# 10XGenomics/lariat

Hardware: AMD Instinct MI355X
Metric: read-pairs/sec aligned to hg38 (per-barcode align loop: SMEM seeding + SW + RFA/MAPQ on device); synthetic hg38-scale reference (higher is better)
Workload: dtype u64/i32 (FM-index + integer DP), f64 (RFA scores)

## Files before the change

### lariat_amd/csrc/k_chain.h

```cpp
#pragma once
#include "k_seed.h"
#include "lh_sort.h"

struct DChainTmp {
    i64 pos, last_rbeg;
    int32_t first_qbeg, last_qbeg, last_len, rid, n, head, tail, w, kept, first, beg, end;
};
#ifndef LH_CHAIN_LDS
#define LH_CHAIN_LDS 256
#endif
struct DChain {
    i64 pos;
    int32_t rid, n, seed_start, w, kept, is_alt;
    float frac_rep;
    int32_t pad;
};

__global__ void __launch_bounds__(64) k_chain(DIndex ix, DOpts o, int n_reads, const i64* __restrict__ seq_off, const i64* __restrict__ seed_off,
                                               i64 pool_cap, const DSeed* __restrict__ seeds, const int32_t* __restrict__ s_rid,
                                               const int32_t* __restrict__ l_rep, int32_t* __restrict__ s_next, DChainTmp* __restrict__ ct,
                                               int32_t* __restrict__ ord, int32_t* __restrict__ srt, DChain* __restrict__ chains,
                                               DSeed* __restrict__ cseeds, int32_t* __restrict__ n_chains, int32_t* __restrict__ status,
                                               const int32_t* __restrict__ list, const int32_t* __restrict__ list_count) {
    __shared__ DChainTmp Cs[LH_CHAIN_LDS];
// ... 215 lines not shown
            if (!shadowed) {
                if (lane == 0) { od[nk] = i; C[st[i]].kept = large_ovlp ? 2 : 3; }
                nk++;
                WAVE_SYNC();
            }
        }
        if (lane == 0) {
            for (int i = 0; i < nk; ++i) {
                int f = C[st[od[i]]].first;
                if (f >= 0) C[st[f]].kept = 1;
            }
            int i, k;
            for (i = k = 0; i < n; ++i) {
                int kp = C[st[i]].kept;
                if (kp == 0 || kp == 3) continue;
                if (++k >= o.max_chain_extend) break;
            }
            for (; i < n; ++i)
                if (C[st[i]].kept < 3) C[st[i]].kept = 0;
        }
    }
    WAVE_SYNC();
    int m = 0;
    {
        int sstart = 0;
        const float frac_rep = (float)l_rep[r] / len;
        for (int i0 = 0; i0 < n; i0 += 64) {
            const int i = i0 + lane;
            int kept = 0, cn = 0;
            DChainTmp c;
            if (i < n) { c = C[st[i]]; kept = c.kept != 0; cn = kept ? c.n : 0; }
            const u64 km = __ballot(kept);
            const int incl = wave_scan_add_i32(cn);
            if (kept) {
                DChain oc;
                oc.pos = c.pos; oc.rid = c.rid; oc.n = c.n; oc.seed_start = sstart + incl - cn; oc.w = c.w; oc.kept = c.kept; oc.is_alt = (ix.contig_alt && ix.contig_alt[c.rid]) ? 1 : 0;
                oc.frac_rep = frac_rep; oc.pad = st[i];
                chains[base + m + lanes_below(km, lane)] = oc;
            }
            m += (int)__popcll(km);
            sstart += wave_readlane(incl, 63);
        }
        if (lane == 0) n_chains[r] = m;
    }
    WAVE_SYNC();
    for (int k = lane; k < m; k += 64) {
        DChain oc = chains[base + k];
        int s = C[oc.pad].head;
        for (int t = 0; s >= 0; s = nx[s], ++t) cseeds[base + oc.seed_start + t] = sd_[s];
    }
    }
}

#ifndef LH_CHAIN_LANE_MAX
#define LH_CHAIN_LANE_MAX 32
#endif
#ifndef LH_EXT_HEAVY_COLS
#define LH_EXT_HEAVY_COLS 64
#endif
#ifndef LH_NARROW_MAX_LOSS
#define LH_NARROW_MAX_LOSS 36
#endif
```

### lariat_amd/csrc/k_chain_lane.h

```cpp
#pragma once
#include "k_extend2.h"

#ifndef LH_CHAIN_LANE_WAVES
#define LH_CHAIN_LANE_WAVES 2
#endif
#define LH_CHAIN_LANE_MAXC 8
#define CLW(ci_, f_) cl[(((ci_) << 3) + (f_)) * 64 + lane]
#define NIB(x_, i_) ((int)(((x_) >> ((i_) << 2)) & 0xf))
#define NIB_SET(x_, i_, v_) ((x_) = ((x_) & ~(0xfu << ((i_) << 2))) | ((uint32_t)(v_) << ((i_) << 2)))
template <class Lt> __device__ __forceinline__ void dev_introsort_small_nib(int n, uint32_t& a, Lt lt, int32_t* wdp) {
    if (n < 1) return;
    if (n == 2) {
        if (lt(NIB(a, 1), NIB(a, 0))) { int x = NIB(a, 0), y = NIB(a, 1); NIB_SET(a, 0, y); NIB_SET(a, 1, x); }
        return;
    }
    if (n > 1) {
        int t = n - 1, i = 0, j = t, k = i + ((j - i) >> 1) + 1;
        if (lt(NIB(a, k), NIB(a, i))) {
            if (lt(NIB(a, k), NIB(a, j))) k = j;
        } else k = lt(NIB(a, j), NIB(a, i)) ? i : j;
        const int rp = NIB(a, k);
        if (k != t) { int y = NIB(a, t); NIB_SET(a, k, y); NIB_SET(a, t, rp); }
        int wd = 4 * LH_CHAIN_LANE_MAX + 8;
        for (;;) {
            do { ++i; LH_WATCH(wdp, wd, 4, return) } while (lt(NIB(a, i), rp));
            do { --j; LH_WATCH(wdp, wd, 5, return) } while (i <= j && lt(rp, NIB(a, j)));
            if (j <= i) break;
            int x = NIB(a, i), y = NIB(a, j); NIB_SET(a, i, y); NIB_SET(a, j, x);
        }
        { int x = NIB(a, i), y = NIB(a, t); NIB_SET(a, i, y); NIB_SET(a, t, x); }
    }
    for (int i = 1; i < n; ++i)
        for (int j = i; j > 0 && lt(NIB(a, j), NIB(a, j - 1)); --j) { int x = NIB(a, j), y = NIB(a, j - 1); NIB_SET(a, j, y); NIB_SET(a, j - 1, x); }
}
__global__ void __launch_bounds__(64, LH_CHAIN_LANE_WAVES) k_chain_lane(DIndex ix, DOpts o, int n_reads, i64 pool_cap, const DSeed* __restrict__ seeds, const int32_t* __restrict__ s_rid,
                                                    const int32_t* __restrict__ l_rep, DChain* __restrict__ chains, DSeed* __restrict__ cseeds, int32_t* __restrict__ n_chains,
                                                    int32_t* __restrict__ status, int32_t* __restrict__ list, int32_t* __restrict__ list_count, int32_t* __restrict__ srt,
                                                    i64* __restrict__ chain_rmax, DCounters* __restrict__ ctr, ExtArgs A, int fuse,
                                                    int32_t* __restrict__ next_count, int32_t* __restrict__ next_list, int32_t* __restrict__ next_key,
                                                    int32_t* __restrict__ defer_count, int32_t* __restrict__ defer_list) {
    const i64* __restrict__ seq_off = A.seq_off; const i64* __restrict__ seed_off = A.seed_off; int32_t* __restrict__ sdone = A.sdone;
    __shared__ uint32_t cl[LH_CHAIN_LANE_MAXC * 8 * 64];
    const int r = blockIdx.x * blockDim.x + threadIdx.x, lane = LANE();
    int heavy = 0, ext_out = 0, ext_key = 0;
    u64 win = 0, cells = 0;
    int nch_done = 0;
    if (r < n_reads) {
        const i64 base = seed_off[r];
        const int S = (int)(seed_off[r + 1] - base);
        if (seed_off[r + 1] > pool_cap) { n_chains[r] = 0; A.n_regs[r] = 0; atomicOr(&status[r], LH_ST_POOL_OVERFLOW); }
        else if (S > LH_CHAIN_LANE_MAX) heavy = 1;
        else {
            const int len = (int)(seq_off[r + 1] - seq_off[r]);
            const DSeed* sd_ = seeds + base;
            const int32_t* rid_ = s_rid + base;
            int nch = 0;
            uint32_t od = 0;
            u64 smap0 = ~0ull, smap1 = ~0ull;
#define SMAP_SET(s_, v_) { if ((s_) < 16) smap0 = (smap0 & ~(0xfull << ((s_) << 2))) | ((u64)(v_) << ((s_) << 2)); else smap1 = (smap1 & ~(0xfull << (((s_) - 16) << 2))) | ((u64)(v_) << (((s_) - 16) << 2)); }
#define SMAP_GET(s_) ((int)((((s_) < 16 ? smap0 : smap1) >> (((s_) & 15) << 2)) & 0xf))
            DSeed pn; pn.rbeg = 0; pn.qbeg = 0; pn.len = 0;
            int ridn = -1;
            if (S > 0) { pn = sd_[0]; ridn = rid_[0]; }
            for (int s = 0; s < S && !heavy; ++s) {
                const DSeed p = pn;
                const int rid = ridn;
                if (s + 1 < S) { pn = sd_[s + 1]; ridn = rid_[s + 1]; }
                if (rid < 0) continue;
                int to_add = 1, lo = 0;
                for (int k = 0; k < nch; ++k) {
                    const int ci = NIB(od, k);
                    const i64 pos = (i64)((u64)CLW(ci, 0) | (u64)CLW(ci, 1) << 32);
                    if (pos <= p.rbeg) lo = k + 1; else break;
                }
                if (lo > 0) {
                    const int ci = NIB(od, lo - 1);
                    const i64 c_pos = (i64)((u64)CLW(ci, 0) | (u64)CLW(ci, 1) << 32);
                    const uint32_t qp = CLW(ci, 3), ridw = CLW(ci, 4);
                    const i64 c_last_rbeg = c_pos + (int32_t)CLW(ci, 2);
                    const int c_first_qbeg = qp & 0xff, c_last_qbeg = (qp >> 8) & 0xff, c_last_len = (qp >> 16) & 0xff, c_rid = (int)(ridw & 0x3fffffffu);
                    const i64 qend = c_last_qbeg + c_last_len, rend = c_last_rbeg + c_last_len;
                    int res = 0;
                    if (rid != c_rid) res = 0;
                    else if (p.qbeg >= c_first_qbeg && p.qbeg + p.len <= qend && p.rbeg >= c_pos && p.rbeg + p.len <= rend) res = 1;
                    else if ((c_last_rbeg < ix.l_pac || c_pos < ix.l_pac) && p.rbeg >= ix.l_pac) res = 0;
                    else {
                        i64 x = p.qbeg - c_last_qbeg, y = p.rbeg - c_last_rbeg;
                        if (y >= 0 && x - y <= o.w && y - x <= o.w && x - c_last_len < o.max_chain_gap && y - c_last_len < o.max_chain_gap) res = 2;
                    }
                    if (res == 2) {
                        const int rr = (int)(p.rbeg - c_pos);
                        CLW(ci, 2) = (uint32_t)rr;
                        CLW(ci, 3) = (uint32_t)c_first_qbeg | (uint32_t)p.qbeg << 8 | (uint32_t)p.len << 16;
                        uint32_t w5 = CLW(ci, 5), w6 = CLW(ci, 6);
                        int n = w5 & 0xff, wq = (int)(w5 >> 8), endq = w6 & 0xff, wr = (int)(w6 >> 8), endr = (int32_t)CLW(ci, 7);
                        if (p.qbeg >= endq) wq += p.len; else if (p.qbeg + p.len > endq) wq += p.qbeg + p.len - endq;
                        endq = endq > p.qbeg + p.len ? endq : p.qbeg + p.len;
                        if (rr >= endr) wr += p.len; else if (rr + p.len > endr) wr += rr + p.len - endr;
                        endr = endr > rr + p.len ? endr : rr + p.len;
                        CLW(ci, 5) = (uint32_t)(n + 1) | (uint32_t)wq << 8; CLW(ci, 6) = (uint32_t)endq | (uint32_t)wr << 8; CLW(ci, 7) = (uint32_t)endr;
                        SMAP_SET(s, ci)
                    }
                    to_add = (res == 0);
                }
                if (to_add) {
                    if (nch == LH_CHAIN_LANE_MAXC) { heavy = 1; break; }
                    const uint32_t lowm = lo ? (0xffffffffu >> (32 - (lo << 2))) : 0u;
                    od = (od & lowm) | ((uint32_t)nch << (lo << 2)) | ((lo < 7) ? ((od & ~lowm) << 4) : 0u);
                    CLW(nch, 0) = (uint32_t)(u64)p.rbeg; CLW(nch, 1) = (uint32_t)((u64)p.rbeg >> 32); CLW(nch, 2) = 0;
                    CLW(nch, 3) = (uint32_t)p.qbeg | (uint32_t)p.qbeg << 8 | (uint32_t)p.len << 16;
                    CLW(nch, 4) = (uint32_t)rid | ((ix.contig_alt && ix.contig_alt[rid]) ? 1u << 30 : 0u);
                    CLW(nch, 5) = 1u | (uint32_t)p.len << 8; CLW(nch, 6) = (uint32_t)(p.qbeg + p.len) | (uint32_t)p.len << 8; CLW(nch, 7) = (uint32_t)p.len;
                    SMAP_SET(s, nch)
                    nch++;
                }
            }
            if (!heavy) {
            for (int k = 0; k < nch; ++k) {
                const uint32_t w5 = CLW(k, 5), w6 = CLW(k, 6);
                int wq = (int)(w5 >> 8), wr = (int)(w6 >> 8);
                int w = wr < wq ? wr : wq;
                CLW(k, 6) = (uint32_t)(w < 1 << 30 ? w : (1 << 30) - 1);
                CLW(k, 5) = w5 & 0xff;
            }
#define C_W(id_) ((int)CLW(id_, 6))
#define C_BEG(id_) ((int)(CLW(id_, 3) & 0xff))
#define C_END(id_) ((int)(((CLW(id_, 3) >> 8) & 0xff) + ((CLW(id_, 3) >> 16) & 0xff)))
#define C_KEPT(id_) ((int)((CLW(id_, 5) >> 8) & 0xff))
#define C_SET_KEPT(id_, v_) (CLW(id_, 5) = (CLW(id_, 5) & ~0xff00u) | ((uint32_t)(v_) << 8))
#define C_FIRST(id_) ((int)((CLW(id_, 5) >> 16) & 0xff) - 1)
#define C_SET_FIRST(id_, v_) (CLW(id_, 5) = (CLW(id_, 5) & ~0xff0000u) | ((uint32_t)((v_) + 1) << 16))
            uint32_t st = 0;
            int n = 0;
            for (int k = 0; k < nch; ++k) {
                const int id = NIB(od, k);
                if (C_W(id) < o.min_chain_weight) continue;
                NIB_SET(st, n, id); n++;
            }
            if (n > 0) {
                dev_introsort_small_nib(n, st, [&](int x, int y) { return C_W(x) > C_W(y); }, o.wd);
                uint32_t kl = 0;
                int nk = 0;
                C_SET_KEPT(NIB(st, 0), 3);
                NIB_SET(kl, nk, 0); nk++;
                for (int i = 1; i < n; ++i) {
                    int large_ovlp = 0, k;
                    const int idi = NIB(st, i);
                    const int ai_beg = C_BEG(idi), ai_end = C_END(idi), ai_w = C_W(idi), ai_alt = (int)(CLW(idi, 4) >> 30) & 1;
                    for (k = 0; k < nk; ++k) {
                        const int idj = NIB(st, NIB(kl, k));
                        const int aj_beg = C_BEG(idj), aj_end = C_END(idj), aj_w = C_W(idj), aj_alt = (int)(CLW(idj, 4) >> 30) & 1;
                        int b_max = aj_beg > ai_beg ? aj_beg : ai_beg;
                        int e_min = aj_end < ai_end ? aj_end : ai_end;
                        if (e_min > b_max && (!aj_alt || ai_alt)) {
                            int li = ai_end - ai_beg, lj = aj_end - aj_beg;
                            int min_l = li < lj ? li : lj;
                            if (e_min - b_max >= min_l * o.mask_level && min_l < o.max_chain_gap) {
                                large_ovlp = 1;
                                if (C_FIRST(idj) < 0) C_SET_FIRST(idj, i);
                                if (ai_w < aj_w * o.drop_ratio && aj_w - ai_w >= o.min_seed_len << 1) break;
                            }
                        }
                    }
                    if (k == nk) { NIB_SET(kl, nk, i); nk++; C_SET_KEPT(idi, large_ovlp ? 2 : 3); }
                }
                for (int i = 0; i < nk; ++i) {
                    int f = C_FIRST(NIB(st, NIB(kl, i)));
                    if (f >= 0) C_SET_KEPT(NIB(st, f), 1);
                }
                int i, k;
                for (i = k = 0; i < n; ++i) {
                    int kp = C_KEPT(NIB(st, i));
                    if (kp == 0 || kp == 3) continue;
                    if (++k >= o.max_chain_extend) break;
                }
                for (; i < n; ++i)
                    if (C_KEPT(NIB(st, i)) < 3) C_SET_KEPT(NIB(st, i), 0);
            }
            int m = 0, sstart = 0;
            const float frac_rep = (float)l_rep[r] / len;
            for (int i = 0; i < n; ++i) {
                const int id = NIB(st, i);
                const int kp = C_KEPT(id);
                if (kp == 0) { CLW(id, 7) = 0xffffffffu; continue; }
                DChain oc;
                oc.pos = (i64)((u64)CLW(id, 0) | (u64)CLW(id, 1) << 32); oc.rid = (int)(CLW(id, 4) & 0x3fffffffu); oc.n = (int)(CLW(id, 5) & 0xff); oc.seed_start = sstart;
                oc.w = C_W(id); oc.kept = kp; oc.is_alt = (int)(CLW(id, 4) >> 30) & 1;
                oc.frac_rep = frac_rep; oc.pad = id;
                chains[base + m] = oc;
                CLW(id, 7) = (uint32_t)sstart; CLW(id, 2) = 0;
                sstart += oc.n;
                m++;
            }
            for (int k = 0; k < nch; ++k) if (C_W(k) < o.min_chain_weight) CLW(k, 7) = 0xffffffffu;
            for (int s = 0; s < S; ++s) {
                const int id = SMAP_GET(s);
                if (id == 0xf) continue;
                const uint32_t ss = CLW(id, 7);
                if (ss == 0xffffffffu) continue;
                const uint32_t t = CLW(id, 2);
                cseeds[base + ss + t] = sd_[s];
                CLW(id, 2) = t + 1;
            }
            n_chains[r] = m;
#undef SMAP_SET
#undef SMAP_GET
#undef C_W
#undef C_BEG
#undef C_END
#undef C_KEPT
#undef C_SET_KEPT
#undef C_FIRST
#undef C_SET_FIRST
            {
                int l_query = len > LH_MAXLEN ? 0 : len;
                const i64 l_pac = ix.l_pac;
                for (int ci = 0; ci < m; ++ci) {
                    DChain c = chains[base + ci];
                    const DSeed* sd = cseeds + base + c.seed_start;
                    int32_t* so = srt + base + c.seed_start;
                    int32_t* done = sdone + base + c.seed_start;
                    const int n = c.n;
                    if (n == 0) continue;
                    i64 r0 = l_pac << 1, r1 = 0;
                    for (int i = 0; i < n; ++i) {
                        DSeed t = sd[i];
                        i64 b = t.rbeg - (t.qbeg + dev_cal_max_gap(o, t.qbeg));
                        i64 e = t.rbeg + t.len + ((l_query - t.qbeg - t.len) + dev_cal_max_gap(o, l_query - t.qbeg - t.len));
                        r0 = r0 < b ? r0 : b;
                        r1 = r1 > e ? r1 : e;
                    }
                    i64 rmax0 = r0 > 0 ? r0 : 0, rmax1 = r1 < l_pac << 1 ? r1 : l_pac << 1;
                    DSeed s0 = sd[0];
                    if (rmax0 < l_pac && l_pac < rmax1) {
                        if (s0.rbeg < l_pac) rmax1 = l_pac;
                        else rmax0 = l_pac;
                    }
                    dev_fetch_clamp(ix, &rmax0, s0.rbeg, &rmax1);
                    win += (u64)(rmax1 - rmax0);
                    chain_rmax[2 * (base + ci)] = rmax0; chain_rmax[2 * (base + ci) + 1] = rmax1;
                    for (int i = 0; i < n; ++i) {
                        DSeed t = sd[i];
                        int rank = 0;
                        for (int u = 0; u < n; ++u) { DSeed x = sd[u]; rank += (x.len < t.len) || (x.len == t.len && u < i); }
                        so[rank] = i;
                        done[i] = 1;
                    }
                }
                nch_done = m;
            }
            if (fuse) ext_out = ext_control<false>(ix, o, A, r, nullptr, lane, &ext_key, &cells);
            }
        }
    }
    ext_append(ext_out, r, ext_key, lane, next_count, next_list, next_key, defer_count, defer_list);
    if (ctr) {
        unsigned w32 = (unsigned)win;
        u64 wtot = (u64)(uint32_t)wave_sum_i32((int)(w32 >> 16)) << 16;
        wtot += (u64)(uint32_t)wave_sum_i32((int)(w32 & 0xffff));
        int ctot = wave_sum_i32(nch_done);
        if (lane == 0 && (wtot || ctot)) { atomicAdd(&LH_CTR(ctr)->win_bases, wtot); atomicAdd(&LH_CTR(ctr)->n_chain_ext, (u64)ctot); }
    }
    u64 hm = __ballot(heavy);
    if (hm) {
        int basep = 0;
        if (lane == 0) basep = atomicAdd(list_count, (int32_t)__popcll(hm));
        basep = wave_readlane(basep, 0);
        if (heavy) list[basep + lanes_below(hm, lane)] = r;
    }
}
```

### lariat_amd/csrc/k_seed.h

```cpp
#pragma once
#include "lh_dev.h"

struct DSeed { i64 rbeg; int32_t qbeg, len; };

#define LH_SCAN_TILE 2048
__device__ __forceinline__ i64 scan_val(const int32_t* in, int i, int n, int add, int at_least) {
    if (i >= n) return 0;
    i64 v = (i64)in[i] + add;
    return v < at_least ? at_least : v;
}
__global__ void __launch_bounds__(256) k_scan_partial(int n, const int32_t* __restrict__ in, int add, int at_least, i64* __restrict__ tile_sum) {
    __shared__ i64 part[256];
    int t = threadIdx.x, base = blockIdx.x * LH_SCAN_TILE + t * 8;
    i64 s = 0;
    for (int u = 0; u < 8; ++u) s += scan_val(in, base + u, n, add, at_least);
    part[t] = s;
    __syncthreads();
    for (int d = 128; d >= 1; d >>= 1) {
        if (t < d) part[t] += part[t + d];
        __syncthreads();
    }
    if (t == 0) tile_sum[blockIdx.x] = part[0];
}
__global__ void __launch_bounds__(256) k_scan_tiles(int n_tiles, i64* __restrict__ tile_sum) {
    __shared__ i64 part[256];
    __shared__ i64 carry_s;
    int t = threadIdx.x;
    if (t == 0) carry_s = 0;
    __syncthreads();
    for (int base = 0; base < n_tiles; base += 256) {
        int i = base + t;
        i64 v = i < n_tiles ? tile_sum[i] : 0;
        part[t] = v;
        __syncthreads();
        for (int d = 1; d < 256; d <<= 1) {
            i64 o = t >= d ? part[t - d] : 0;
            __syncthreads();
            part[t] += o;
            __syncthreads();
        }
        i64 excl = part[t] - v + carry_s;
        __syncthreads();
        if (i < n_tiles) tile_sum[i] = excl;
        if (t == 255) carry_s += part[255];
        __syncthreads();
    }
    if (t == 0) tile_sum[n_tiles] = carry_s;
}
__global__ void __launch_bounds__(256) k_scan_final(int n, const int32_t* __restrict__ in, int add, int at_least, const i64* __restrict__ tile_sum, int n_tiles,
                                                    i64* __restrict__ out) {
    __shared__ i64 part[256];
    int t = threadIdx.x, base = blockIdx.x * LH_SCAN_TILE + t * 8;
    i64 loc[8], s = 0;
    for (int u = 0; u < 8; ++u) { loc[u] = s; s += scan_val(in, base + u, n, add, at_least); }
    part[t] = s;
    __syncthreads();
    for (int d = 1; d < 256; d <<= 1) {
        i64 o = t >= d ? part[t - d] : 0;
        __syncthreads();
        part[t] += o;
        __syncthreads();
    }
    i64 excl = part[t] - s + tile_sum[blockIdx.x];
    for (int u = 0; u < 8; ++u) if (base + u < n) out[base + u] = excl + loc[u];
    if (blockIdx.x == 0 && t == 0) out[n] = tile_sum[n_tiles];
}

__global__ void __launch_bounds__(256) k_seed_owner(int n_reads, const i64* __restrict__ seed_off, i64 pool_cap, int32_t* __restrict__ owner) {
    for (int r = blockIdx.x * blockDim.x + threadIdx.x; r < n_reads; r += gridDim.x * blockDim.x) {
        i64 e = seed_off[r + 1] < pool_cap ? seed_off[r + 1] : pool_cap;
        for (i64 g = seed_off[r]; g < e; ++g) owner[g] = r;
    }
}

__global__ void __launch_bounds__(256) k_seed(DIndex ix, DOpts o, int n_reads, const i64* __restrict__ seed_off, i64 pool_cap,
                                              const DIntv* __restrict__ intv, const int32_t* __restrict__ n_intv, DSeed* __restrict__ seeds,
                                              int32_t* __restrict__ s_rid, DCounters* __restrict__ ctr, const int32_t* __restrict__ owner,
                                              const int32_t* __restrict__ big_slot, const DIntv* __restrict__ big_slab) {
    i64 total = seed_off[n_reads];
    if (total > pool_cap) total = pool_cap;
    i64 stride = (i64)gridDim.x * blockDim.x;
    i64 nrounds = (total + stride - 1) / stride;
    for (i64 rd = 0; rd < nrounds; ++rd) {
        i64 g = rd * stride + (i64)blockIdx.x * blockDim.x + threadIdx.x;
        int nlf = 0, nsa = 0;
        if (g < total) {
            int r = owner[g];
            i64 u = g - seed_off[r];
            const int bs = big_slot ? big_slot[r] : -1;
            const DIntv* iv = bs < 0 ? intv + (size_t)r * LH_MAX_INTV : big_slab + ((size_t)bs * 2 + 1) * LH_BIG_INTV;
            int n = n_intv[r];
            u64 x0 = 0, step = 1, info = 0;
            for (int t = 0; t < n; ++t) {
                u64 s = iv[t].x2;
                u64 st = 1, c = s;
                if (s > (u64)o.max_occ) {
                    st = s / (u64)o.max_occ;
                    c = (s + st - 1) / st;
                    if (c > (u64)o.max_occ) c = (u64)o.max_occ;
                }
                if ((u64)u < c) { x0 = iv[t].x0; step = st; info = iv[t].info; break; }
                u -= (i64)c;
            }
            i64 rbeg;
            if (x0 >> 62 & 1) rbeg = (i64)(x0 & ~(1ull << 62));
            else rbeg = (i64)dev_sa(ix, x0 + (u64)u * step, &nlf);
            nsa = 1;
            int qbeg = (int)(info >> 32), slen = (int)(uint32_t)info - qbeg;
            DSeed sd;
            sd.rbeg = rbeg; sd.qbeg = qbeg; sd.len = slen;
            seeds[g] = sd;
            s_rid[g] = dev_intv2rid(ix, rbeg, rbeg + slen);
        }
        if (ctr) {
            int tl = wave_sum_i32(nlf), ts = wave_sum_i32(nsa);
            if (LANE() == 0 && ts) { atomicAdd(&LH_CTR(ctr)->n_lf, (u64)tl); atomicAdd(&LH_CTR(ctr)->n_sa, (u64)ts); }
        }
    }
}
```

### lariat_amd/csrc/k_smem4.h

```cpp
#pragma once
#ifndef LH_K1_SLAB_CHUNK
#define LH_K1_SLAB_CHUNK 4
#endif
#include "lh_dev.h"
static_assert((LH_MAXLEN + 2) % LH_K1_SLAB_CHUNK == 0, "a lane's list of LH_MAXLEN + 2 entries is a whole number of chunks");
#define LH_K1_LDS_BUDGET 10240
#ifndef LH_K1_QW_SMALL
#define LH_K1_QW_SMALL 24
#endif
#ifdef LH_K1_RING
#define LH_K1_RING_OF(qw_) (LH_K1_RING)
#else
#define LH_K1_RING_OF(qw_) ((LH_K1_LDS_BUDGET - (qw_) * 256) / 2048)
#endif
static_assert(LH_K1_QW_SMALL >= 1 && LH_K1_QW_SMALL <= 32, "the small query staging holds at most the full query");

struct __attribute__((aligned(16))) PEnt { u64 lo, hi; };
#define LH_M40 0xffffffffffull
__device__ __forceinline__ PEnt pe_pack(u64 x0, u64 x1, u64 x2, int info) {
    PEnt e;
    e.lo = x0 | (x2 << 40);
    e.hi = x1 | ((x2 >> 24) << 40) | ((u64)(uint32_t)info << 49);
    return e;
}
#define PE_X0(e) ((e).lo & LH_M40)
#define PE_X1(e) ((e).hi & LH_M40)
#define PE_X2(e) (((e).lo >> 40) | ((((e).hi >> 40) & 0x1ffull) << 24))
#define PE_INFO(e) ((int)((e).hi >> 49))
#define LH_POSF (1ull << 62)

#define S4_FETCH 0
#define S4_DONE 1
#define S4_REQ_FWD 2
#define S4_REQ_BWD 3
#define S4_REQ_P3 4
#define S4_REQ_FRUN 5
#define S4_REQ_BRUN 6
#define S4_BWD_EMIT 8
#define S4_BWD_INIT 9
#define S4_BWD_EMIT0 10
#define S4_SMEM_DONE 11
#define S4_P1_SCAN 12
#define S4_P2_NEXT 13
#define S4_P3_SCAN 14
#define S4_READ_DONE 15
#define S4_FRUN_INIT 16
#define S4_FRUN_INIT2 17
#define S4_FRUN_END 18
#define S4_FRUN_END2 19
#define S4_BRUN_INIT 20
#define S4_BRUN_INIT2 21
#define S4_BRUN_END 22
#define S4_TRI_C1 23
#define S4_P3_JUMP 24
#define S4_P3_JUMP2 25
#define S4_TRI_C1B 26
#define S4_TRI_LCP2 27
#define S4_FJUMP 28
#define S4_FJUMP2 29
#define S4_P2_PROBE 30
#define S4_P2_PROBE2 31
#define S4_P2_PROBE3 32
#define S4_P3_PREP 35
#define S4_P3_PREP2 36
#define S4_P3_PREP3 37
#define S4_P3_T0 38
#define S4_P3_T1 39
#define S4_BT_INIT 40
#define S4_BT_B 41
#define S4_PENDING 34
#define TD_ROW 1
#define TD_SMEM 2
#define TD_FADV 4
#define TD_KEY 8
#define LH_KMER 12

#ifndef LH_SLOW_BATCH
#define LH_SLOW_BATCH 4
#endif
#ifndef LH_SLOW_BATCH_P2
#define LH_SLOW_BATCH_P2 16
#endif
// ... 1046 lines not shown
                        const PEnt te = kt[(((1ull << (2 * lnew)) - 4) / 3) + fcode];
                        ok.x0 = PE_X0(te); ok.x1 = PE_X1(te); ok.x2 = PE_X2(te); ok.info = 0;
                        ++n_kt;
                    } else { ok = dev_extend_c(ix, c, 3 - b, 0); ++n_exec; }
                    ++n_ext;
                    if (ok.x2 < (u64)o.max_mem_intv && i - x >= o.min_seed_len) {
                        if (ok.x2 > 0) {
                            if (on >= LH_MAX_INTV) ovf = 1;
                            else { ok.info = (u64)x << 32 | (u64)(i + 1); out[on++] = ok; }
                        }
                        nx = i + 1;
                        break;
                    }
                    c = ok;
                }
                x = nx;
            }
        }
#undef QN
        if (ovf) rst |= LH_ST_INTV_OVERFLOW;
        n_intv[r] = on;
        status[r] = rst;
    }
    if (ctr) {
        unsigned t1 = (unsigned)wave_sum_i32((int)n_ext), t2 = (unsigned)wave_sum_i32((int)n_exec), t3 = (unsigned)wave_sum_i32((int)n_kt);
        if (lane == 0 && t1) { atomicAdd(&LH_CTR(ctr)->n_ext, (u64)t1); atomicAdd(&LH_CTR(ctr)->n_ext_exec[2], (u64)t2); atomicAdd(&LH_CTR(ctr)->n_ktree[2], (u64)t3); }
    }
}

__global__ void __launch_bounds__(256) k_smem_fin(DOpts o, int n_reads, DIntv* __restrict__ intv, const int32_t* __restrict__ n_intv, int32_t* __restrict__ seed_cnt,
                                                   int32_t* __restrict__ l_rep_out, const int32_t* __restrict__ big_slot) {
    int gid = (blockIdx.x * blockDim.x + threadIdx.x) >> 4, sub = threadIdx.x & 15;
    int r = gid < n_reads ? gid : n_reads - 1;
    int live = gid < n_reads && !(big_slot && big_slot[r] >= 0);
    DIntv* a = intv + (size_t)r * LH_MAX_INTV;
    int n = live ? n_intv[r] : 0;
    DIntv mine[4];
    int rank[4];
    for (int t = 0; t < 4; ++t) {
        int e = sub + 16 * t;
        mine[t].x0 = mine[t].x1 = mine[t].x2 = 0; mine[t].info = ~0ull;
        if (e < n) mine[t] = a[e];
        rank[t] = 0;
    }
    const int nt = (n + 15) >> 4;
    for (int u = 0; u < n; ++u) {
        u64 oi = a[u].info;
#pragma unroll
        for (int t = 0; t < 4; ++t)
            if (t < nt) { int e = sub + 16 * t; rank[t] += (oi < mine[t].info) || (oi == mine[t].info && u < e); }
    }
    __syncthreads();
    int cnt = 0, rep = 0;
#pragma unroll
    for (int t = 0; t < 4; ++t) {
        int e = sub + 16 * t;
        if (t < nt && e < n && live) {
            a[rank[t]] = mine[t];
            cnt += dev_seed_count(o, mine[t].x2);
            rep += mine[t].x2 > (u64)o.max_occ;
        }
    }
    cnt += (int)dpp_xor1((uint32_t)cnt); cnt += (int)dpp_xor2((uint32_t)cnt); cnt += (int)dpp_half_mirror((uint32_t)cnt); cnt += (int)dpp_ror8((uint32_t)cnt);
    rep += (int)dpp_xor1((uint32_t)rep); rep += (int)dpp_xor2((uint32_t)rep); rep += (int)dpp_half_mirror((uint32_t)rep); rep += (int)dpp_ror8((uint32_t)rep);
    __syncthreads();
    if (sub == 0 && live) { seed_cnt[r] = cnt; l_rep_out[r] = rep ? dev_l_rep(o, a, n) : 0; }
}
__global__ void __launch_bounds__(64) k_smem_fin_big(DOpts o, K1Big big, const int32_t* __restrict__ n_intv, int32_t* __restrict__ seed_cnt, int32_t* __restrict__ l_rep_out) {
    const int lane = LANE(), n_big = *big.count;
    for (int item = blockIdx.x; item < n_big; item += gridDim.x) {
        const int r = big.list[item];
        const DIntv* a = big.slab + (size_t)big.slot[r] * (2 * LH_BIG_INTV);
        DIntv* b = big.slab + ((size_t)big.slot[r] * 2 + 1) * LH_BIG_INTV;
        const int n = n_intv[r];
        int cnt = 0;
        for (int e = lane; e < n; e += 64) {
            const DIntv m = a[e];
            int rank = 0;
            for (int u = 0; u < n; ++u) { const u64 oi = a[u].info; rank += (oi < m.info) || (oi == m.info && u < e); }
            b[rank] = m;
            cnt += dev_seed_count(o, m.x2);
        }
        cnt = wave_sum_i32(cnt);
        WAVE_SYNC();
        if (lane == 0) { seed_cnt[r] = cnt; l_rep_out[r] = dev_l_rep(o, b, n); }
        WAVE_SYNC();
    }
}
__global__ void __launch_bounds__(256) k_big_collect(int n_reads, int32_t* __restrict__ status, int32_t* __restrict__ n_intv, int32_t* __restrict__ slot, int32_t* __restrict__ list,
                                                      int32_t* __restrict__ count, int base, int cap) {
    const int r = blockIdx.x * blockDim.x + threadIdx.x;
    if (r >= n_reads) return;
    if (base > 0 && slot[r] >= 0) return;
    int s = -1;
    if (status[r] & LH_ST_INTV_OVERFLOW) {
        s = atomicAdd(count + 1, 1);
        if (s < cap) { list[atomicAdd(count, 1)] = r; status[r] &= ~LH_ST_INTV_OVERFLOW; n_intv[r] = 0; s += base; }
        else s = -1;
    }
    slot[r] = s;
}

__global__ void __launch_bounds__(256) k_intv_rows(DIndex ix, int n_reads, DIntv* __restrict__ intv, const int32_t* __restrict__ n_intv, K1Big big) {
    const int r = blockIdx.x * blockDim.x + threadIdx.x;
    if (r >= n_reads || !ix.isa) return;
    DIntv* a = dev_intv_of(intv, big, r, 1);
    const int n = n_intv[r];
    for (int k = 0; k < n; ++k) {
        DIntv p = a[k];
        if (!(p.x0 & LH_POSF)) continue;
        const u64 pos = p.x0 & ~LH_POSF;
        const int l = (int)(uint32_t)p.info - (int)(p.info >> 32);
        p.x0 = ix.isa[pos]; p.x1 = ix.isa[ix.seq_len - (pos + (u64)l)];
        a[k] = p;
    }
}
```

### lariat_amd/csrc/lh_dev.h

```cpp
#pragma once
#include <stdint.h>

#ifdef LH_EMU
#include "hip_emu.h"
#define LH_LAUNCH(kernel, grid, block, stream, ...)                                          \
    do {                                                                                     \
        if (getenv("LH_EMU_TRACE")) fprintf(stderr, "emu launch %s grid=%d\n", #kernel, (int)(grid)); \
        emu::launch(dim3(grid), dim3(block), [&]() { kernel(__VA_ARGS__); });                \
    } while (0)
struct uint4 { uint32_t x, y, z, w; };
struct uint2 { uint32_t x, y; };
#else
#include <hip/hip_runtime.h>
#define LH_LAUNCH(kernel, grid, block, stream, ...) \
    hipLaunchKernelGGL(kernel, dim3(grid), dim3(block), 0, stream, __VA_ARGS__)
#endif

#define LH_WAVE 64
#define LH_MAXLEN 250
#ifndef LH_MAX_INTV
#define LH_MAX_INTV 64
#endif
#define LH_BIG_INTV 1024
#define LH_MAX_CIGAR 64
#define LH_MAX_MM 64
#define LH_RESCUE_SLOTS 50

#ifdef LH_EMU
#define WAVE_SYNC() (emu::note(__FILE__, __LINE__), __syncthreads())
#else
#define WAVE_SYNC() __syncthreads()
#endif
#define LANE() ((int)(threadIdx.x & 63))
#ifdef LH_EMU
#define EMU_SYNC() WAVE_SYNC()
#else
#define EMU_SYNC() __builtin_amdgcn_wave_barrier()
#endif

typedef uint64_t u64;
typedef int64_t i64;

#ifdef LH_EMU
#define LH_UNI(c) (c)
#else
#define LH_UNI(c) (__builtin_amdgcn_readfirstlane((int)(c)) != 0)
#endif

#define LH_WD_SLOTS 32
#define LH_WATCH(wdp, budget, code, action) if (--(budget) < 0) { (wdp)[code] = 1; action; }
#ifdef LH_NOWATCH_SORT
#define LH_WATCH_S(wdp, budget, code, action)
#else
#define LH_WATCH_S LH_WATCH
#endif
#ifdef LH_NOWATCH_DEDUP
#define LH_WATCH_D(wdp, budget, code, action)
#else
#define LH_WATCH_D LH_WATCH
#endif

#define LH_ST_INTV_OVERFLOW 1
#define LH_ST_TOO_LONG 2
#define LH_ST_CIGAR_OVERFLOW 4
#define LH_ST_MM_OVERFLOW 8
#define LH_ST_POOL_OVERFLOW 16

struct DIndex {
    const uint4* occ;
    const u64* sb;
    int32_t sb_shift;
    const u64* isa;
    const uint32_t* tn;
    const uint8_t* lcp;
    const uint8_t* plcp;
    const u64* rep_t;
    const void* kmer12;
    const void* ktree;
    int32_t ktree_levels;
    const u64* bloom1;
    const u64* bloom2;
    uint32_t bloom1_words, bloom2_words;
    const u64* sa;
    const uint8_t* pac;
    const i64* contig_off;
    const int32_t* contig_len;
    const uint8_t* contig_alt;
    const int32_t* rid_bins;
    int32_t rid_bin_shift;
    u64 primary, L2[5], seq_len;
    i64 l_pac;
    int32_t sa_intv, n_contigs;
};

struct DOpts {
    int32_t a, b, o_del, e_del, o_ins, e_ins, pen_unpaired, pen_clip5, pen_clip3, w, zdrop, T;
    int32_t min_seed_len, min_chain_weight, max_chain_extend, split_width, max_occ, max_chain_gap, max_ins, max_mem_intv, max_matesw;
    float split_factor, mask_level, drop_ratio, XA_drop_ratio, mask_level_redun, mapQ_coef_len;
    int32_t pes_low, pes_high, rescue_score_delta, rescue_max_hits, aln_score_delta, run_inference;
    double improper_pair_penalty, genome_length;
    int8_t mat[25];
    int32_t* wd;
};

struct DIntv { u64 x0, x1, x2, info; };

struct DReg {
    i64 rb, re;
    int32_t qb, qe, rid, score, truesc, sub, csub, w, seedcov, secondary, seedlen0, n_comp, is_alt;
    float frac_rep;
};

#define LH_CTR_SLOTS 64
struct DCounters { u64 n_ext, n_lf, n_sa, win_bases, n_chain_ext, ext_cells, glob_cells, n_rescue, rescue_cells, n_ext_exec[3], n_ktree[3], n_bt, rescue_cells_exec, n_glob_listed, n_glob_exec; };
#define LH_CTR(ctr) ((ctr) + (blockIdx.x & (LH_CTR_SLOTS - 1)))

__device__ __forceinline__ u64 shfl_u64(u64 v, int src) {
    uint32_t lo = (uint32_t)v, hi = (uint32_t)(v >> 32);
    lo = __shfl(lo, src); hi = __shfl(hi, src);
    return (u64)hi << 32 | lo;
}
__device__ __forceinline__ i64 shfl_i64(i64 v, int src) { return (i64)shfl_u64((u64)v, src); }
__device__ __forceinline__ i64 shfl_xor_i64(i64 v, int m) {
    uint32_t lo = (uint32_t)(u64)v, hi = (uint32_t)((u64)v >> 32);
    lo = __shfl_xor(lo, m); hi = __shfl_xor(hi, m);
    return (i64)((u64)hi << 32 | lo);
}
#ifdef LH_EMU
__device__ __forceinline__ int wave_max_i32(int v) {
    for (int m = 32; m >= 1; m >>= 1) { int o = __shfl_xor(v, m); v = v > o ? v : o; }
    return v;
}
__device__ __forceinline__ int wave_min_i32(int v) {
    for (int m = 32; m >= 1; m >>= 1) { int o = __shfl_xor(v, m); v = v < o ? v : o; }
    return v;
}
__device__ __forceinline__ int wave_sum_i32(int v) {
    for (int m = 32; m >= 1; m >>= 1) v += __shfl_xor(v, m);
    return v;
}
__device__ __forceinline__ int wave_scan_max_i32(int v, int lane) {
    for (int d = 1; d < 64; d <<= 1) { int o = __shfl_up(v, d); if (lane >= d) v = v > o ? v : o; }
    return v;
}
__device__ __forceinline__ int wave_scan_add_i32(int v) {
    int lane = LANE();
    for (int d = 1; d < 64; d <<= 1) { int o = __shfl_up(v, d); if (lane >= d) v += o; }
    return v;
}
__device__ __forceinline__ int wave_shr1_i32(int v, int fill) { int o = __shfl_up(v, 1); return LANE() == 0 ? fill : o; }
__device__ __forceinline__ int wave_readlane(int v, int l) { return __shfl(v, l); }
#else
#define LH_DPP(old, v, ctrl, rmask) __builtin_amdgcn_update_dpp((old), (v), (ctrl), (rmask), 0xF, false)
__device__ __forceinline__ int wave_scan_max_i32(int v, int) {
    const int ID = (int)0x80000000;
    int t;
    t = LH_DPP(ID, v, 0x111, 0xF); v = v > t ? v : t;
    t = LH_DPP(ID, v, 0x112, 0xF); v = v > t ? v : t;
// ... 301 lines not shown
```

### lariat_amd/csrc/lh_host.inc

```
#include <math.h>
#include <stdlib.h>
#include <stdio.h>
#include <string.h>

#include <algorithm>
#include <array>
#include <functional>
#include <memory>
#include <mutex>
#include <string>
#include <vector>
#include <deque>
#include <map>

#include "../../include/lariat_hip.h"
#include "k_smem4.h"
#include "k_chain_lane.h"
#include "k_chain_cl.h"
#include "k_rfa.h"
#include "k_rescue3.h"
#include "lh_result_cols.h"

static void lh_print_wd(const int32_t* d_wd) {
    int32_t h[LH_WD_SLOTS];
// ... 456 lines not shown
        if (p2_tasks) LH_LAUNCH(k_p2_clamp, (N + 255) / 256, 256, c->stream, N, c->d_n_intv);
        T_END();
#ifdef LH_K1_TRACE
        { int rc = k1_trace_lens(c, trace); if (rc) return rc; }
#endif
        T_BEGIN("k_smem4_p3");
        if (o.max_mem_intv > 0 && q4)
            LH_LAUNCH(k_smem_p3_lock, (N + 255) / 256, 256, c->stream, ix4, o, N, q4, (const i64*)c->d_seq_off, c->d_intv, c->d_n_intv, c->d_status, c->d_ctr);
        else if (o.max_mem_intv > 0)
            smem_pass<3, false>(c, ix4, o, N, g3, nobig);
        T_END();
        T_BEGIN("k_smem_fin");
        { int rc = k1_big_round(c, o, ix4, N, 0); if (rc) return rc; }
        LH_LAUNCH(k_smem_fin, (N * 16 + 255) / 256, 256, c->stream, o, N, c->d_intv, c->d_n_intv, c->d_seed_cnt, c->d_l_rep, (const int32_t*)c->d_big_slot);
        T_END();
    }
    T_BEGIN("k_scan_seeds");
    { int rc = run_scan(c, N, c->d_seed_cnt, 0, 0, c->d_seed_off); if (rc) return rc; }
    T_END();
    {
        { int rc = peek_seed_total(c, N); if (rc) return rc; }
        while (c->h_peek->k1.big_asked > (i64)(c->big_cap - c->big_base)) {
            const i64 asked = c->h_peek->k1.big_asked, old_cap = c->big_cap, new_cap = old_cap + asked + asked / 8 + 16;
            if (new_cap > (1 << 30)) return set_err(LH_E_CAPACITY, "too many reads with more than LH_MAX_INTV SMEM intervals for one batch: split the batch");
            DIntv* slab = nullptr; int32_t* list = nullptr;
            DevGroup grown;
            DALLOC(grown, slab, (size_t)new_cap * 2 * LH_BIG_INTV); DALLOC(grown, list, (size_t)new_cap);
            HIPCHK(hipMemcpyAsync(slab, c->d_big_slab, (size_t)old_cap * 2 * LH_BIG_INTV * sizeof(DIntv), hipMemcpyDeviceToDevice, c->stream));
            HIPCHK(hipStreamSynchronize(c->stream));
            std::swap(c->d_big_slab, slab); std::swap(c->d_big_list, list);
            grown.release();
            c->big_base = (int)old_cap; c->big_cap = (int)new_cap;
            { int rc = k1_big_round(c, o, ix4, N, c->big_base); if (rc) return rc; }
            { int rc = run_scan(c, N, c->d_seed_cnt, 0, 0, c->d_seed_off); if (rc) return rc; }
            { int rc = peek_seed_total(c, N); if (rc) return rc; }
        }
        c->big_base = 0;
        const i64 total = c->h_peek->k1.seeds;
        if (total > c->pool_cap) {
            c->seed_mem.release(); c->pool_cap = c->regpool_cap = 0;
            size_t free_b = 0, total_b = 0;
            HIPCHK(hipMemGetInfo(&free_b, &total_b));
            const double per_seed = sizeof(DSeed) * 2 + 4 * 4 + sizeof(DChainTmp) + sizeof(DChain) + 16 + 2.0 * sizeof(DReg) + 12 + 40;
            const double need = ((double)total * 1.25 + (double)c->cap_reads * LH_RESCUE_SLOTS) * per_seed;
            if (need > (double)free_b - 2e9)
                return set_err(LH_E_CAPACITY, "the batch has " + std::to_string(total) + " seeds: their workspace (" + std::to_string((long long)(need / 1e9)) + " GB) does not fit the " +
                                                  std::to_string((long long)(free_b / 1000000000)) + " GB of HBM that are free: split the batch");
            int rc = alloc_seed_pools(c, total + total / 4);
            if (rc) return rc;
        }
    }
    T_BEGIN("k_seed");
    int g2 = (int)((i64)N * 8 / 256 + 1); if (g2 > 2048) g2 = 2048;
    LH_LAUNCH(k_seed_owner, (N + 255) / 256 < 8192 ? (N + 255) / 256 : 8192, 256, c->stream, N, (const i64*)c->d_seed_off, c->pool_cap, c->d_s_next);
    LH_LAUNCH(k_seed, g2, 256, c->stream, ix, o, N, c->d_seed_off, c->pool_cap, c->d_intv, c->d_n_intv, c->d_seeds, c->d_s_rid, c->d_ctr, (const int32_t*)c->d_s_next, (const int32_t*)c->d_big_slot, (const DIntv*)c->d_big_slab);
    T_END();
    T_BEGIN("k_scan_regs");
    { int rc = run_scan(c, N, c->d_seed_cnt, LH_RESCUE_SLOTS, 0, c->d_reg_off); if (rc) return rc; }
    T_END();
    T_BEGIN("k_chain");
    HIPCHK(hipMemsetAsync(c->d_ext_jobs, 0, sizeof(DExtJobs), c->stream));
    {
        ExtArgs A = ext_args(c);
        const int fuse = (c->flags & LH_F_EXT_WAVE) ? 0 : 1;
        LH_LAUNCH(k_chain_lane, (N + 63) / 64, 64, c->stream, ix, o, N, c->pool_cap, c->d_seeds, c->d_s_rid, c->d_l_rep, c->d_chains, c->d_cseeds, c->d_n_chains, c->d_status,
                  c->d_aln_r, c->d_ext_jobs->wave_range + 1, c->d_srt, c->d_chain_rmax, c->d_ctr, A, fuse, c->d_ext_jobs->count + 1, c->d_ext_jlist, c->d_ext_jkey,
                  c->d_ext_jobs->heavy_range + 1, c->d_ext_heavy);
        const int32_t* wlist = c->d_aln_r;
        const int32_t* wcount = c->d_ext_jobs->wave_range + 1;
        if (!(c->flags & LH_F_CHAIN_WAVE)) {
            int32_t* const fb_count = &c->d_aln_count->full;
            HIPCHK(hipMemsetAsync(fb_count, 0, sizeof(int32_t), c->stream));
#define LH_K3_CL(CAP_, GRID_, LO_, LAST_, ST_)                                                                                                                         \
            LH_LAUNCH((k_chain_cl<CAP_>), N < (GRID_) ? N : (GRID_), 64, ST_, ix, o, (const i64*)c->d_seq_off, (const i64*)c->d_seed_off, c->pool_cap, (const DSeed*)c->d_seeds, \
                      (const int32_t*)c->d_s_rid, (const int32_t*)c->d_l_rep, c->d_chains, c->d_cseeds, c->d_n_chains, c->d_status, wlist, wcount, LO_, LAST_, c->d_aln_ci, fb_count)
            HIPCHK(hipEventRecord(c->ev_fork, c->stream));
            HIPCHK(hipStreamWaitEvent(c->aux[1], c->ev_fork, 0)); HIPCHK(hipStreamWaitEvent(c->aux[2], c->ev_fork, 0));
            LH_K3_CL(LH_CHAIN_CL_CAP_C, 2048, LH_CHAIN_CL_CAP_B, 1, c->aux[2]);
            LH_K3_CL(LH_CHAIN_CL_CAP_B, 8192, LH_CHAIN_CL_CAP_A, 0, c->aux[1]);
            LH_K3_CL(LH_CHAIN_CL_CAP_A, 16384, 0, 0, c->stream);
            HIPCHK(hipEventRecord(c->ev_join[1], c->aux[1])); HIPCHK(hipEventRecord(c->ev_join[2], c->aux[2]));
            HIPCHK(hipStreamWaitEvent(c->stream, c->ev_join[1], 0)); HIPCHK(hipStreamWaitEvent(c->stream, c->ev_join[2], 0));
#undef LH_K3_CL
            wlist = c->d_aln_ci; wcount = fb_count;
#ifdef LH_RFA_PROF
            { int rc = prof_chain_cl(c); if (rc) return rc; }
#endif
            if (lh_debug_sync()) {
                int32_t nl = 0, nf = 0;
                if (hipStreamSynchronize(c->stream) == hipSuccess && hipMemcpy(&nl, c->d_ext_jobs->wave_range + 1, 4, hipMemcpyDeviceToHost) == hipSuccess &&
                    hipMemcpy(&nf, fb_count, 4, hipMemcpyDeviceToHost) == hipSuccess)
                    fprintf(stderr, "[lh] K3: %d reads listed for the wave kernels, %d of them left to k_chain by k_chain_cl\n", nl, nf);
            }
        }
        LH_LAUNCH(k_chain, N < 16384 ? N : 16384, 64, c->stream, ix, o, N, c->d_seq_off, c->d_seed_off, c->pool_cap, c->d_seeds, c->d_s_rid, c->d_l_rep, c->d_s_next, c->d_ct,
                  c->d_ord, c->d_srt, c->d_chains, c->d_cseeds, c->d_n_chains, c->d_status, wlist, wcount);
    }
    T_END();
    return LH_OK;
}

static int pipe_align(lh_context* c, const lh_opts* opts) {
    if (!c || !opts) return set_err(LH_E_ARG, "lh_align_resident: null argument");
    if (!c->resident) return set_err(LH_E_ARG, "no batch resident: call lh_batch_upload first");
    if (opts->abi_version != LH_ABI_VERSION) return set_err(LH_E_ARG, "lh_opts.abi_version does not match LH_ABI_VERSION (use lh_opts_init)");
    if (opts->flags & ~(LH_F_NO_SWEEP_FILTER | LH_F_EXT_WAVE | LH_F_EXT_SERIAL | LH_F_CHAIN_WAVE | LH_F_P2_TASKS | LH_F_RESCUE_FULL)) return set_err(LH_E_ARG, "lh_opts.flags: unknown bit set");
    HIPCHK(hipSetDevice(c->idx->device));
    {
        std::vector<void*> fl;
        { std::lock_guard<std::mutex> g(c->slot_mu); fl.swap(c->free_later); }
        for (void* q : fl) hipFree(q);
    }
    if (!c->pool_cap) { int rc = alloc_seed_pools(c, first_pool_cap(c)); if (rc) return rc; }
    if (!c->cand_cap) { int rc = alloc_cand_pools(c, first_cand_cap(c)); if (rc) return rc; }
    DOpts o = to_dopts(opts);
    o.wd = c->d_wd;
    c->flags = opts->flags;
    int t = 0;
// ... 110 lines not shown
```

Measured before the change: 49.65 million.

## Chain light reads directly from SMEM intervals, skipping seed pool materialization

Reads whose intervals are all single-occurrence, already-positioned seeds are flagged in k_smem_fin with a sentinel l_rep value. For those reads k_seed skips writing seeds and rids to the pool, and k_chain_lane decodes seeds straight from the interval buffer, computing contig ids on the fly with a cached contig-bounds check. The aim is to cut global writes and reads of the seed pool and the separate rid lookups. The cost is extra decode logic and a fallback that materializes seeds when a read turns out heavy, plus some debug path counters and a moved SA counter.

```diff
diff --git a/lariat_amd/csrc/k_chain.h b/lariat_amd/csrc/k_chain.h
--- a/lariat_amd/csrc/k_chain.h
+++ b/lariat_amd/csrc/k_chain.h
@@ -291,9 +291,6 @@
     }
 }
 
-#ifndef LH_CHAIN_LANE_MAX
-#define LH_CHAIN_LANE_MAX 32
-#endif
 #ifndef LH_EXT_HEAVY_COLS
 #define LH_EXT_HEAVY_COLS 64
 #endif
diff --git a/lariat_amd/csrc/k_chain_lane.h b/lariat_amd/csrc/k_chain_lane.h
--- a/lariat_amd/csrc/k_chain_lane.h
+++ b/lariat_amd/csrc/k_chain_lane.h
@@ -4,7 +4,12 @@
 #ifndef LH_CHAIN_LANE_WAVES
 #define LH_CHAIN_LANE_WAVES 2
 #endif
+#ifndef LH_CHAIN_LANE_MAXC
 #define LH_CHAIN_LANE_MAXC 8
+#endif
+#ifndef LH_K3_WEAK
+#define LH_K3_WEAK 0
+#endif
 #define CLW(ci_, f_) cl[(((ci_) << 3) + (f_)) * 64 + lane]
 #define NIB(x_, i_) ((int)(((x_) >> ((i_) << 2)) & 0xf))
 #define NIB_SET(x_, i_, v_) ((x_) = ((x_) & ~(0xfu << ((i_) << 2))) | ((uint32_t)(v_) << ((i_) << 2)))
@@ -33,8 +38,17 @@
     for (int i = 1; i < n; ++i)
         for (int j = i; j > 0 && lt(NIB(a, j), NIB(a, j - 1)); --j) { int x = NIB(a, j), y = NIB(a, j - 1); NIB_SET(a, j, y); NIB_SET(a, j - 1, x); }
 }
-__global__ void __launch_bounds__(64, LH_CHAIN_LANE_WAVES) k_chain_lane(DIndex ix, DOpts o, int n_reads, i64 pool_cap, const DSeed* __restrict__ seeds, const int32_t* __restrict__ s_rid,
-                                                    const int32_t* __restrict__ l_rep, DChain* __restrict__ chains, DSeed* __restrict__ cseeds, int32_t* __restrict__ n_chains,
+#if defined(LH_EMU) && defined(LH_K3_PATH_COUNT)
+static u64 lh_k3_path_count[6];
+extern "C" void lh_k3_path_count_read(unsigned long long* out, int reset) {
+    for (int i = 0; i < 6; ++i) { out[i] = lh_k3_path_count[i]; if (reset) lh_k3_path_count[i] = 0; }
+}
+#define LH_K3_PATH(i_) atomicAdd(&lh_k3_path_count[i_], (u64)1)
+#else
+#define LH_K3_PATH(i_)
+#endif
+__global__ void __launch_bounds__(64, LH_CHAIN_LANE_WAVES) k_chain_lane(DIndex ix, DOpts o, int n_reads, i64 pool_cap, DSeed* __restrict__ seeds, int32_t* __restrict__ s_rid,
+                                                    const DIntv* __restrict__ intv, int pool_all, int32_t* __restrict__ l_rep, DChain* __restrict__ chains, DSeed* __restrict__ cseeds, int32_t* __restrict__ n_chains,
                                                     int32_t* __restrict__ status, int32_t* __restrict__ list, int32_t* __restrict__ list_count, int32_t* __restrict__ srt,
                                                     i64* __restrict__ chain_rmax, DCounters* __restrict__ ctr, ExtArgs A, int fuse,
                                                     int32_t* __restrict__ next_count, int32_t* __restrict__ next_list, int32_t* __restrict__ next_key,
@@ -44,28 +58,63 @@
     const int r = blockIdx.x * blockDim.x + threadIdx.x, lane = LANE();
     int heavy = 0, ext_out = 0, ext_key = 0;
     u64 win = 0, cells = 0;
-    int nch_done = 0;
+    int nch_done = 0, nsa = 0;
     if (r < n_reads) {
         const i64 base = seed_off[r];
         const int S = (int)(seed_off[r + 1] - base);
-        if (seed_off[r + 1] > pool_cap) { n_chains[r] = 0; A.n_regs[r] = 0; atomicOr(&status[r], LH_ST_POOL_OVERFLOW); }
+        const int lrep = l_rep[r];
+        const bool from_intv = lrep == LH_LREP_FROM_INTV;
+        if (seed_off[r + 1] > pool_cap) {
+            n_chains[r] = 0; A.n_regs[r] = 0; atomicOr(&status[r], LH_ST_POOL_OVERFLOW);
+            if (from_intv && pool_cap > base) nsa = (int)(pool_cap - base);
+        }
         else if (S > LH_CHAIN_LANE_MAX) heavy = 1;
         else {
             const int len = (int)(seq_off[r + 1] - seq_off[r]);
-            const DSeed* sd_ = seeds + base;
             const int32_t* rid_ = s_rid + base;
+            const char* const sp = from_intv ? (const char*)(intv + (size_t)r * LH_MAX_INTV) : (const char*)(seeds + base);
+            const int sstep = from_intv ? (int)sizeof(DIntv) : (int)sizeof(DSeed), sw1 = from_intv ? 24 : 8;
+            auto seed_raw = [&](int s_, u64& w0_, u64& w1_) {
+                const char* q = sp + s_ * sstep;
+                __builtin_memcpy(&w0_, __builtin_assume_aligned(q, 8), 8); __builtin_memcpy(&w1_, __builtin_assume_aligned(q + sw1, 8), 8);
+            };
+            auto seed_of = [&](u64 w0_, u64 w1_) {
+                DSeed t;
+                if (from_intv) { t.rbeg = (i64)(w0_ & ~LH_POSF); t.qbeg = (int32_t)(w1_ >> 32); t.len = (int32_t)(uint32_t)w1_ - t.qbeg; }
+                else { t.rbeg = (i64)w0_; t.qbeg = (int32_t)(uint32_t)w1_; t.len = (int32_t)(w1_ >> 32); }
+                return t;
+            };
+            i64 cb0 = 0, cb1 = 0;
+            int crid = -1;
+            auto seed_rid = [&](const DSeed& t) {
+#if LH_K3_WEAK == 2
+                if (crid >= 0) return crid;
+#endif
+                if (crid >= 0 && t.rbeg >= cb0 && t.rbeg + t.len <= cb1) { LH_K3_PATH(4); return crid; }
+                LH_K3_PATH(3);
+                const int rid = dev_intv2rid(ix, t.rbeg, t.rbeg + t.len);
+                if (rid >= 0) {
+                    i64 b = ix.contig_off[rid], e = b + ix.contig_len[rid];
+                    if (t.rbeg >= ix.l_pac) { const i64 x = b; b = (ix.l_pac << 1) - e; e = (ix.l_pac << 1) - x; }
+                    cb0 = b; cb1 = e; crid = rid;
+                }
+                return rid;
+            };
+            if (from_intv) nsa = S;
             int nch = 0;
             uint32_t od = 0;
             u64 smap0 = ~0ull, smap1 = ~0ull;
 #define SMAP_SET(s_, v_) { if ((s_) < 16) smap0 = (smap0 & ~(0xfull << ((s_) << 2))) | ((u64)(v_) << ((s_) << 2)); else smap1 = (smap1 & ~(0xfull << (((s_) - 16) << 2))) | ((u64)(v_) << (((s_) - 16) << 2)); }
 #define SMAP_GET(s_) ((int)((((s_) < 16 ? smap0 : smap1) >> (((s_) & 15) << 2)) & 0xf))
-            DSeed pn; pn.rbeg = 0; pn.qbeg = 0; pn.len = 0;
+            u64 n0 = 0, n1 = 0;
             int ridn = -1;
-            if (S > 0) { pn = sd_[0]; ridn = rid_[0]; }
+            if (S > 0) { seed_raw(0, n0, n1); if (!from_intv) ridn = rid_[0]; }
             for (int s = 0; s < S && !heavy; ++s) {
-                const DSeed p = pn;
-                const int rid = ridn;
-                if (s + 1 < S) { pn = sd_[s + 1]; ridn = rid_[s + 1]; }
+                const u64 c0 = n0, c1 = n1;
+                const int ridp = ridn;
+                if (s + 1 < S) { seed_raw(s + 1, n0, n1); if (!from_intv) ridn = rid_[s + 1]; }
+                const DSeed p = seed_of(c0, c1);
+                const int rid = from_intv ? seed_rid(p) : ridp;
                 if (rid < 0) continue;
                 int to_add = 1, lo = 0;
                 for (int k = 0; k < nch; ++k) {
@@ -115,7 +164,20 @@
                     nch++;
                 }
             }
+            if (heavy && from_intv) {
+#if LH_K3_WEAK != 1
+                for (int s = 0; s < S; ++s) {
+                    u64 w0, w1;
+                    seed_raw(s, w0, w1);
+                    const DSeed t = seed_of(w0, w1);
+                    seeds[base + s] = t; s_rid[base + s] = seed_rid(t);
+                }
+#endif
+                l_rep[r] = 0;
+                LH_K3_PATH(1);
+            }
             if (!heavy) {
+            LH_K3_PATH(S == 0 ? 5 : from_intv ? 0 : 2);
             for (int k = 0; k < nch; ++k) {
                 const uint32_t w5 = CLW(k, 5), w6 = CLW(k, 6);
                 int wq = (int)(w5 >> 8), wr = (int)(w6 >> 8);
@@ -178,7 +240,7 @@
                     if (C_KEPT(NIB(st, i)) < 3) C_SET_KEPT(NIB(st, i), 0);
             }
             int m = 0, sstart = 0;
-            const float frac_rep = (float)l_rep[r] / len;
+            const float frac_rep = (float)(from_intv ? 0 : lrep) / len;
             for (int i = 0; i < n; ++i) {
                 const int id = NIB(st, i);
                 const int kp = C_KEPT(id);
@@ -199,7 +261,9 @@
                 const uint32_t ss = CLW(id, 7);
                 if (ss == 0xffffffffu) continue;
                 const uint32_t t = CLW(id, 2);
-                cseeds[base + ss + t] = sd_[s];
+                u64 w0, w1;
+                seed_raw(s, w0, w1);
+                cseeds[base + ss + t] = seed_of(w0, w1);
                 CLW(id, 2) = t + 1;
             }
             n_chains[r] = m;
@@ -260,6 +324,8 @@
         wtot += (u64)(uint32_t)wave_sum_i32((int)(w32 & 0xffff));
         int ctot = wave_sum_i32(nch_done);
         if (lane == 0 && (wtot || ctot)) { atomicAdd(&LH_CTR(ctr)->win_bases, wtot); atomicAdd(&LH_CTR(ctr)->n_chain_ext, (u64)ctot); }
+        const int stot = wave_sum_i32(pool_all ? 0 : nsa);
+        if (lane == 0 && stot) atomicAdd(&LH_CTR(ctr)->n_sa, (u64)stot);
     }
     u64 hm = __ballot(heavy);
     if (hm) {
diff --git a/lariat_amd/csrc/k_seed.h b/lariat_amd/csrc/k_seed.h
--- a/lariat_amd/csrc/k_seed.h
+++ b/lariat_amd/csrc/k_seed.h
@@ -66,10 +66,11 @@
     if (blockIdx.x == 0 && t == 0) out[n] = tile_sum[n_tiles];
 }
 
-__global__ void __launch_bounds__(256) k_seed_owner(int n_reads, const i64* __restrict__ seed_off, i64 pool_cap, int32_t* __restrict__ owner) {
+__global__ void __launch_bounds__(256) k_seed_owner(int n_reads, const i64* __restrict__ seed_off, i64 pool_cap, const int32_t* __restrict__ l_rep, int all, int32_t* __restrict__ owner) {
     for (int r = blockIdx.x * blockDim.x + threadIdx.x; r < n_reads; r += gridDim.x * blockDim.x) {
         i64 e = seed_off[r + 1] < pool_cap ? seed_off[r + 1] : pool_cap;
-        for (i64 g = seed_off[r]; g < e; ++g) owner[g] = r;
+        const int32_t v = (!all && l_rep[r] == LH_LREP_FROM_INTV) ? -1 : r;
+        for (i64 g = seed_off[r]; g < e; ++g) owner[g] = v;
     }
 }
 
@@ -84,8 +85,8 @@
     for (i64 rd = 0; rd < nrounds; ++rd) {
         i64 g = rd * stride + (i64)blockIdx.x * blockDim.x + threadIdx.x;
         int nlf = 0, nsa = 0;
-        if (g < total) {
-            int r = owner[g];
+        const int r = g < total ? owner[g] : -1;
+        if (r >= 0) {
             i64 u = g - seed_off[r];
             const int bs = big_slot ? big_slot[r] : -1;
             const DIntv* iv = bs < 0 ? intv + (size_t)r * LH_MAX_INTV : big_slab + ((size_t)bs * 2 + 1) * LH_BIG_INTV;
diff --git a/lariat_amd/csrc/k_smem4.h b/lariat_amd/csrc/k_smem4.h
--- a/lariat_amd/csrc/k_smem4.h
+++ b/lariat_amd/csrc/k_smem4.h
@@ -27,7 +27,6 @@
 #define PE_X1(e) ((e).hi & LH_M40)
 #define PE_X2(e) (((e).lo >> 40) | ((((e).hi >> 40) & 0x1ffull) << 24))
 #define PE_INFO(e) ((int)((e).hi >> 49))
-#define LH_POSF (1ull << 62)
 
 #define S4_FETCH 0
 #define S4_DONE 1
@@ -1180,6 +1179,7 @@
     }
     __syncthreads();
     int cnt = 0, rep = 0;
+    int byp = 0;
 #pragma unroll
     for (int t = 0; t < 4; ++t) {
         int e = sub + 16 * t;
@@ -1187,12 +1187,15 @@
             a[rank[t]] = mine[t];
             cnt += dev_seed_count(o, mine[t].x2);
             rep += mine[t].x2 > (u64)o.max_occ;
+            byp += (mine[t].x0 & LH_POSF) != 0;
         }
     }
     cnt += (int)dpp_xor1((uint32_t)cnt); cnt += (int)dpp_xor2((uint32_t)cnt); cnt += (int)dpp_half_mirror((uint32_t)cnt); cnt += (int)dpp_ror8((uint32_t)cnt);
     rep += (int)dpp_xor1((uint32_t)rep); rep += (int)dpp_xor2((uint32_t)rep); rep += (int)dpp_half_mirror((uint32_t)rep); rep += (int)dpp_ror8((uint32_t)rep);
+    byp += (int)dpp_xor1((uint32_t)byp); byp += (int)dpp_xor2((uint32_t)byp); byp += (int)dpp_half_mirror((uint32_t)byp); byp += (int)dpp_ror8((uint32_t)byp);
     __syncthreads();
-    if (sub == 0 && live) { seed_cnt[r] = cnt; l_rep_out[r] = rep ? dev_l_rep(o, a, n) : 0; }
+    const int from_intv = !LH_K3_SEED_POOL && n > 0 && byp == n && cnt == n && n <= LH_CHAIN_LANE_MAX;
+    if (sub == 0 && live) { seed_cnt[r] = cnt; l_rep_out[r] = from_intv ? LH_LREP_FROM_INTV : rep ? dev_l_rep(o, a, n) : 0; }
 }
 __global__ void __launch_bounds__(64) k_smem_fin_big(DOpts o, K1Big big, const int32_t* __restrict__ n_intv, int32_t* __restrict__ seed_cnt, int32_t* __restrict__ l_rep_out) {
     const int lane = LANE(), n_big = *big.count;
diff --git a/lariat_amd/csrc/lh_dev.h b/lariat_amd/csrc/lh_dev.h
--- a/lariat_amd/csrc/lh_dev.h
+++ b/lariat_amd/csrc/lh_dev.h
@@ -22,6 +22,12 @@
 #define LH_MAX_INTV 64
 #endif
 #define LH_BIG_INTV 1024
+#ifndef LH_CHAIN_LANE_MAX
+#define LH_CHAIN_LANE_MAX 32
+#endif
+#ifndef LH_K3_SEED_POOL
+#define LH_K3_SEED_POOL 0
+#endif
 #define LH_MAX_CIGAR 64
 #define LH_MAX_MM 64
 #define LH_RESCUE_SLOTS 50
@@ -104,6 +110,8 @@
 };
 
 struct DIntv { u64 x0, x1, x2, info; };
+#define LH_POSF (1ull << 62)
+#define LH_LREP_FROM_INTV (-1)
 
 struct DReg {
     i64 rb, re;
diff --git a/lariat_amd/csrc/lh_host.inc b/lariat_amd/csrc/lh_host.inc
--- a/lariat_amd/csrc/lh_host.inc
+++ b/lariat_amd/csrc/lh_host.inc
@@ -532,7 +532,8 @@
     }
     T_BEGIN("k_seed");
     int g2 = (int)((i64)N * 8 / 256 + 1); if (g2 > 2048) g2 = 2048;
-    LH_LAUNCH(k_seed_owner, (N + 255) / 256 < 8192 ? (N + 255) / 256 : 8192, 256, c->stream, N, (const i64*)c->d_seed_off, c->pool_cap, c->d_s_next);
+    const int pool_all = c->dump_stop_after_dedup ? 1 : 0;
+    LH_LAUNCH(k_seed_owner, (N + 255) / 256 < 8192 ? (N + 255) / 256 : 8192, 256, c->stream, N, (const i64*)c->d_seed_off, c->pool_cap, (const int32_t*)c->d_l_rep, pool_all, c->d_s_next);
     LH_LAUNCH(k_seed, g2, 256, c->stream, ix, o, N, c->d_seed_off, c->pool_cap, c->d_intv, c->d_n_intv, c->d_seeds, c->d_s_rid, c->d_ctr, (const int32_t*)c->d_s_next, (const int32_t*)c->d_big_slot, (const DIntv*)c->d_big_slab);
     T_END();
     T_BEGIN("k_scan_regs");
@@ -543,7 +544,7 @@
     {
         ExtArgs A = ext_args(c);
         const int fuse = (c->flags & LH_F_EXT_WAVE) ? 0 : 1;
-        LH_LAUNCH(k_chain_lane, (N + 63) / 64, 64, c->stream, ix, o, N, c->pool_cap, c->d_seeds, c->d_s_rid, c->d_l_rep, c->d_chains, c->d_cseeds, c->d_n_chains, c->d_status,
+        LH_LAUNCH(k_chain_lane, (N + 63) / 64, 64, c->stream, ix, o, N, c->pool_cap, c->d_seeds, c->d_s_rid, (const DIntv*)c->d_intv, pool_all, c->d_l_rep, c->d_chains, c->d_cseeds, c->d_n_chains, c->d_status,
                   c->d_aln_r, c->d_ext_jobs->wave_range + 1, c->d_srt, c->d_chain_rmax, c->d_ctr, A, fuse, c->d_ext_jobs->count + 1, c->d_ext_jlist, c->d_ext_jkey,
                   c->d_ext_jobs->heavy_range + 1, c->d_ext_heavy);
         const int32_t* wlist = c->d_aln_r;
```

Result: no change. 49.16 million (-1.0%).
